# pathint/RankCompV3.jl

Hardware: AMD Instinct MI355X
Metric: gene-pair·sample comparisons/sec at 20k genes × 1k samples (higher is better)
Workload: dtype u16

## Files before the change

### rankcompv3.jl_amd/_ffi.py

```python
from __future__ import annotations

import ctypes
import os
import subprocess
from typing import NamedTuple

import numpy as np

_HERE = os.path.dirname(os.path.abspath(__file__))
LIB_PATH = os.environ.get("REO_LIB_PATH") or os.path.join(_HERE, "libreo_hip.so")
CSRC = os.path.join(_HERE, "csrc")

REO_OK, REO_EINVAL, REO_EHIP, REO_ECOMM, REO_ENOMEM = 0, -1, -2, -3, -4
NTIMINGS = 12

SYMBOLS = [
    "reo_version", "reo_last_error", "reo_create", "reo_destroy", "reo_trim_memory", "reo_set_shard", "reo_set_allreduce", "reo_set_allgather",
    "reo_create_multi", "reo_comm_unique_id", "reo_comm_init_rank",
    "reo_set_matrix_f64", "reo_set_matrix_i64", "reo_set_matrix_dev_f64", "reo_set_matrix_dev_i64",
    "reo_set_matrix_f32", "reo_set_matrix_i32", "reo_set_matrix_dev_f32", "reo_set_matrix_dev_i32",
    "reo_set_matrix_rm_f64", "reo_set_matrix_rm_i64", "reo_set_matrix_rm_f32", "reo_set_matrix_rm_i32",
    "reo_set_matrix_csc_f64", "reo_set_matrix_csc_i64", "reo_set_matrix_csc_f32", "reo_set_matrix_csc_i32",
    "reo_set_groups", "reo_compute_thresholds", "reo_set_thresholds", "reo_get_thresholds", "reo_threshold",
    "reo_build_pairs", "reo_pair_counts", "reo_get_codes", "reo_tally", "reo_identify_degs", "reo_mccullagh",
# ... 551 lines not shown
        out = np.zeros((cont.shape[0], 5), dtype=np.float64)
        check(self._L.reo_mccullagh(self._h, _ptr(cont), cont.shape[0], _ptr(out)))
        return out

    @staticmethod
    def _pseudobulk_args(cells, order, chunk_ptr):
        order = np.ascontiguousarray(order, dtype=np.int32)
        chunk_ptr = np.ascontiguousarray(chunk_ptr, dtype=np.int32)
        n_out = chunk_ptr.size - 1
        if hasattr(cells, "tocsc"):
            m = cells.tocsc()
            m.sort_indices()
            G, C = m.shape
            isint = np.issubdtype(m.dtype, np.integer)
            val = np.ascontiguousarray(m.data, dtype=np.int64 if isint else np.float64)
            colptr = np.ascontiguousarray(m.indptr, dtype=np.int64)
            rowidx = np.ascontiguousarray(m.indices, dtype=np.int32)
            args = (G, C, _ptr(colptr), _ptr(rowidx), _ptr(val), _ptr(order), order.size, _ptr(chunk_ptr), n_out)
            return "csc", "i64" if isint else "f64", args, G, (m, val, colptr, rowidx, order, chunk_ptr)
        X = np.asarray(cells)
        isint = np.issubdtype(X.dtype, np.integer)
        Xf = np.asfortranarray(X, dtype=np.int64 if isint else np.float64)
        G, C = Xf.shape
        args = (_ptr(Xf), G, C, G, _ptr(order), order.size, _ptr(chunk_ptr), n_out)
        return "dense", "i64" if isint else "f64", args, G, (Xf, order, chunk_ptr)

    def pseudobulk(self, cells, order, chunk_ptr) -> np.ndarray:
        form, ty, args, G, keep = self._pseudobulk_args(cells, order, chunk_ptr)
        out = np.zeros((G, args[-1]), dtype=np.int64 if ty == "i64" else np.float64, order="F")
        check(getattr(self._L, f"reo_pseudobulk_{form}_{ty}")(self._h, *args, _ptr(out)))
        return out

    def set_matrix_pseudobulk(self, cells, order, chunk_ptr) -> None:
        if is_device_sparse(cells) or is_device_tensor(cells):
            order = np.ascontiguousarray(order, dtype=np.int32)
            chunk_ptr = np.ascontiguousarray(chunk_ptr, dtype=np.int32)
            n_out = chunk_ptr.size - 1
            tail = (_ptr(order) if order.size else None, order.size, _ptr(chunk_ptr), n_out)
            if is_device_sparse(cells):
                ty, G, C, nnz, colptr, rowidx, val, bits, keep = device_csc_entry(cells)
                check(getattr(self._L, "reo_set_matrix_pseudobulk_csc_dev_" + ty)(self._h, G, C, nnz, _dptr(colptr), _dptr(rowidx), bits, _dptr(val), *tail))
            else:
                ptr, G, C, ld, ty, keep = device_matrix(cells)
                check(getattr(self._L, "reo_set_matrix_pseudobulk_dense_dev_" + ty)(self._h, ctypes.c_void_p(ptr), G, C, ld, *tail))
            self.G, self.S = G, n_out
            return
        form, ty, args, G, keep = self._pseudobulk_args(cells, order, chunk_ptr)
        check(getattr(self._L, f"reo_set_matrix_pseudobulk_{form}_{ty}")(self._h, *args))
        self.G, self.S = G, args[-1]

    def filter_matrix(self, min_profiles: int = 0, min_features: int = 0):
        info = self.info()
        pk = np.zeros(info["S"], dtype=np.uint8)
        gk = np.zeros(info["G"], dtype=np.uint8)
        sk, gkn = ctypes.c_int64(0), ctypes.c_int64(0)
        check(self._L.reo_filter_matrix(self._h, int(min_profiles), int(min_features), _ptr(pk) if pk.size else None, _ptr(gk) if gk.size else None,
                                        ctypes.byref(sk), ctypes.byref(gkn)))
        self.G, self.S = int(gkn.value), int(sk.value)
        return pk.astype(bool), gk.astype(bool)

    def get_matrix(self) -> np.ndarray:
        info = self.info()
        dt = {1: np.float64, 2: np.int64, 3: np.float32}.get(info["resident_dtype"])
        if dt is None:
            raise DimensionMismatch(REO_EINVAL, "no expression matrix set")
        out = np.zeros((info["G"], info["S"]), dtype=dt, order="F")
        check(self._L.reo_get_matrix(self._h, _ptr(out), out.nbytes))
        return out

    def set_profiling(self, on: bool) -> None:
        check(self._L.reo_set_profiling(self._h, 1 if on else 0))

    def reset_timings(self) -> None:
        check(self._L.reo_reset_timings(self._h))

    def timings(self) -> dict:
        ms = np.zeros(NTIMINGS, dtype=np.float64)
        check(self._L.reo_get_timings(self._h, _ptr(ms), NTIMINGS))
        return {"transform_ms": ms[0], "k1_ms": ms[1], "k2_ms": ms[2], "iter_ms": ms[3], "k3_ms": max(ms[3] - ms[2], 0.0), "k2_launches": int(ms[4]),
                "k1_launches": int(ms[5]), "exchange_ms": ms[6], "pseudobulk_ms": ms[7], "k2_full_ms": ms[8],
                "k2_full_launches": int(ms[9]), "k2_delta_ms": ms[10], "set_matrix_host_wall_ms": ms[11]}

    def info(self) -> dict:
        v = np.zeros(28, dtype=np.int64)
        check(self._L.reo_get_info(self._h, _ptr(v), 28))
        return {"G": int(v[0]), "S": int(v[1]), "Gp": int(v[2]), "table_bytes": int(v[3]), "has_ties": int(v[4]),
                "tiles_owned": int(v[5]), "tiles_total": int(v[6]), "tile_i": int(v[7]), "chunk_j": int(v[8]),
                "chunks_per_panel": int(v[9]), "unit_h": int(v[10]), "sample_slots": int(v[11]),
                "shared_group_counts": int(v[12]), "group_count_bytes": int(v[13]), "transform_in_lds": int(v[14]), "xcc_local_histograms": int(v[15]),
                "cycle_period": int(v[16]), "cycle_found_at_pass": int(v[17]), "cycle_passes_skipped": int(v[18]), "upload_link_bytes": int(v[19]),
                "eager_range_launches": int(v[20]), "rowmajor_upload": int(v[21]),
                "csc_upload": int(v[22]), "csc_nnz": int(v[23]), "resident_dtype": int(v[24]),
                "k1_slot_order": int(v[25]), "k1_half_tiles_separated": int(v[26]), "csc_device": int(v[27])}
```

### rankcompv3.jl_amd/csrc/api.hip

```cpp
#include <execinfo.h>
#include <signal.h>
#include <unistd.h>

#include <ctime>
#include <algorithm>
#include <chrono>
#include <cmath>
#include <cstdarg>
#include <cstdio>
#include <cstdlib>
#include <cstring>

#include "pair_list.h"
#include "reo_internal.h"
#include "sample_counts.h"
#include "upload_csc.h"

#include <mutex>
#include <unordered_map>

namespace reo {

static thread_local std::string g_err;
thread_local bool tl_release_synced = false;
// ... 503 lines not shown
    } else {
        set_error("the persistent iteration kernel gave up at a grid barrier (a workgroup did not arrive within its bound); "
                  "REO_LIGHT=1 runs the same passes as separate launches");
    }
    return REO_EHIP;
}

static int32_t need_complete_table(reo_ctx *c)
{
    if (c->built_k < 0) { set_error("no class table: call reo_build_pairs first"); return REO_EINVAL; }
    if (!c->table_complete) {
        set_error("shard %d of %d holds only its own part of the class table: attach a communicator (reo_comm_init_rank) or an "
                  "exchange hook (reo_set_allgather, reo_set_allreduce) before reo_build_pairs", c->rank, c->world);
        return REO_ECOMM;
    }
    return REO_OK;
}

}

using namespace reo;

extern "C" {

int32_t reo_version(void) { return 700; }

int32_t reo_trim_memory(void)
{
    std::vector<Block> all;
    {
        Pool &P = pool();
        std::lock_guard<std::mutex> lk(P.mu);
        all.swap(P.free_blocks);
        P.cached = 0;
    }
    int dev = 0;
    const bool have_dev = hipGetDevice(&dev) == hipSuccess;
    for (const Block &b : all) {
        if (!b.pinned) (void)hipSetDevice(b.device);
        raw_free(b.p, b.pinned);
    }
    {
        Handles &H = handles();
        std::lock_guard<std::mutex> lk(H.mu);
        for (int k = 0; k < 2; ++k) {
            for (auto &st : H.streams[k]) { (void)hipSetDevice(st.first); (void)hipStreamDestroy(st.second); }
            for (auto &ev : H.events[k]) { (void)hipSetDevice(ev.first); (void)hipEventDestroy(ev.second); }
            H.streams[k].clear(); H.events[k].clear();
        }
    }
    if (have_dev) (void)hipSetDevice(dev);
    return REO_OK;
}

const char *reo_last_error(void) { return g_err.c_str(); }

int32_t reo_create(reo_ctx **out, int32_t device, uint64_t seed)
{
    if (!out) { set_error("out is null"); return REO_EINVAL; }
    *out = nullptr;
    if (getenv("REO_DEBUG_SEGV")) install_segv_backtrace();
    int ndev = 0;
    if (hipGetDeviceCount(&ndev) != hipSuccess || ndev == 0) {
        set_error("no HIP device visible: libreo_hip has no CPU fallback");
        return REO_EHIP;
    }
    if (device < 0) REO_HIP_CHECK(hipGetDevice(&device));
    if (device >= ndev) { set_error("device %d out of range (%d visible)", device, ndev); return REO_EINVAL; }
    hipDeviceProp_t prop;
    REO_HIP_CHECK(hipGetDeviceProperties(&prop, device));
    if (strncmp(prop.gcnArchName, "gfx950", 6) != 0) {
        set_error("device %d is %s; this library carries gfx950 (MI355X) code objects only", device, prop.gcnArchName);
        return REO_EHIP;
    }
    REO_HIP_CHECK(hipSetDevice(device));
    reo_ctx *c = new (std::nothrow) reo_ctx();
    if (!c) { set_error("out of host memory"); return REO_ENOMEM; }
    c->device = device;
    c->seed = seed;
    if (const char *e = getenv("REO_K1_WAVE")) c->k1_wave = (e[0] != '0');
    if (const char *e = getenv("REO_K1_HALF")) c->k1_half = (e[0] != '0');
    if (const char *e = getenv("REO_K1_SLOTS")) c->k1_slots = (e[0] != '0');
    if (const char *e = getenv("REO_K1_QUEUE")) c->k1_queue = (e[0] != '0');
    if (const char *e = getenv("REO_K1_WORKERS")) c->k1_workers = std::max(1, atoi(e));
    if (const char *e = getenv("REO_K1_ORDER")) c->k1_order = std::max(0, std::min(2, atoi(e)));
    {
        int n = 0;
        if (hipDeviceGetAttribute(&n, hipDeviceAttributeMultiprocessorCount, c->device) == hipSuccess && n > 0) c->n_cus = n;
    }
    if (const char *e = getenv("REO_SPIN_WAIT")) c->spin_wait = (e[0] != '0');
    if (const char *e = getenv("REO_CHECK_HOOK_TABLE")) c->check_hook_table = (e[0] != '0');
    if (const char *e = getenv("REO_SHARE_GROUP_COUNTS")) c->share_counts = (e[0] != '0');
    if (const char *e = getenv("REO_LIGHT_BAND")) c->light_band = std::max(0, atoi(e));
    if (const char *e = getenv("REO_HIST_BELOW")) c->hist_below = std::max(0, atoi(e));
    if (const char *e = getenv("REO_CYCLE")) c->cycle_watch = atoi(e) != 0;
    if (const char *e = getenv("REO_LIGHT")) c->light_mode = e[0] == '0' ? 0 : (e[0] == '2' ? 2 : (e[0] == '3' ? 3 : 1));
    c->light_window = light_window(); c->light_min_g = light_min_genes();
    if (const char *e = getenv("REO_LIGHT_WINDOW")) c->light_window = std::max(1, std::min(31, atoi(e)));
    if (const char *e = getenv("REO_LIGHT_MIN_G")) c->light_min_g = std::max(64, atoi(e));
    if (const char *e = getenv("REO_STATE_MIRROR")) c->state_mirror_wanted = (e[0] != '0');
    if (const char *e = getenv("REO_EXCHANGE_WAVES")) c->x_waves = std::max(1, std::min(8, atoi(e)));
    if (const char *e = getenv("REO_EAGER_UPLOAD")) c->eager_mode = std::max(0, std::min(2, atoi(e)));
    if (const char *e = getenv("REO_EAGER_CHUNK")) c->eager_chunk = std::max(1, atoi(e));
    if (const char *e = getenv("REO_EAGER_GATE")) c->eager_gate = atoi(e) != 0;
    if (const char *e = getenv("REO_EAGER_RANGES")) c->eager_ranges = std::max(1, std::min(6, atoi(e)));
    if (const char *e = getenv("REO_UPLOAD_THREADS")) c->upload_threads = std::max(0, std::min(64, atoi(e)));
    c->debug_passes = getenv("REO_DEBUG_PASSES") != nullptr;
    c->debug_stamps = getenv("REO_DEBUG_STAMPS") != nullptr;
    c->k1_stamps = getenv("REO_K1_STAMPS") != nullptr;
    hipError_t e = handle_stream(&c->stream, 0);
    if (e != hipSuccess) { delete c; set_error("hipStreamCreate failed: %s", hipGetErrorString(e)); return REO_EHIP; }
    int ok = 0;
    const char *xe = getenv("REO_XCC_LOCAL");
    if (!(xe && xe[0] == '0')) {
        const int32_t rc = xcc_selftest(c, &ok);
        if (rc) { reo_destroy(c); return rc; }
    }
    c->xcc_local = ok;
    *out = c;
    return REO_OK;
}

void reo_destroy(reo_ctx *c)
{
    if (!c) return;
    for (reo_ctx *p : c->peers) reo_destroy(p);
    c->peers.clear();
    (void)hipSetDevice(c->device);
    for (int q = 0; q < 2; ++q) if (c->k1s[q]) (void)hipStreamSynchronize(c->k1s[q]);
    if (c->xs) (void)hipStreamSynchronize(c->xs);
    if (c->up) (void)hipStreamSynchronize(c->up);
    if (c->rk) (void)hipStreamSynchronize(c->rk);
    (void)hipStreamSynchronize(c->stream);
    comm_release(c);
    collect_timings(c);
    tl_release_synced = true;
    for (auto &t : c->pool) { release_event(t.a, 1); release_event(t.b, 1); }
    c->dX_owned.release(); c->pos.release(); c->lo.release(); c->hi.release(); c->goff_dev.release();
    c->table.release();
    c->t_kin.release(); c->t_kout.release(); c->t_vin.release(); c->t_vout.release(); c->t_temp.release();
    c->t_order.release(); c->t_flags.release(); c->t_slots.release(); c->unit_map.release();
    for (auto &il : c->k1_wave_items) il.buf.release();
    for (int q = 0; q < 2; ++q) { release_stream(c->k1s[q], 0); release_event(c->ev_k1_join[q], 0); }
    release_stream(c->xs, 0);
    release_stream(c->up, 0);
    release_stream(c->rk, 1);
    for (auto &e : c->ev_rk) release_event(e, 0);
    for (auto &e : c->ev_up) release_event(e, 0);
    c->e_lists.release();
    for (int q = 0; q < 3; ++q) {
        if (c->stage_h[q]) pool_free(c->stage_h[q], c->stage_cap, true);
        c->stage_d[q].release();
        release_event(c->ev_stage[q], 0);
        release_event(c->ev_widen[q], 0);
    }
    release_event(c->ev_fork, 0);
    release_event(c->ev_x, 0);
    for (auto &e : c->ev_k1) release_event(e, 0);
    c->t_pos16.release(); c->t_lo16.release(); c->t_hi16.release(); c->gcounts.release();
    c->k1_slot_part.release(); c->k1_slot_maps.release(); c->pos_s.release(); c->lo_s.release(); c->k1_queue_ctr.release();
    c->t_pos32.release(); c->t_lo32.release(); c->t_hi32.release(); c->t_vin32.release(); c->t_vout32.release();
    for (int t = 0; t < 2; ++t) { c->refbits[t].release(); c->refbytes[t].release(); }
    c->raw.release(); c->delta_list.release(); c->cont.release(); c->result.release(); c->sorted_d.release(); c->sorted_p.release();
    c->rank_s.release(); c->rank_a.release(); c->scal.release(); c->blockmin.release();
    c->state.release(); c->trace.release(); c->modes.release(); c->cand.release(); c->hist.release(); c->mrank.release(); c->lstate.release(); c->clist.release(); c->olist.release(); c->units_all.release(); c->xsend.release(); c->xrecv.release(); c->check_flag.release(); c->gridbar.release(); c->chunk_v.release(); c->chunk_i.release(); c->part.release();
    if (c->host_state) pool_free(c->host_state, sizeof(IterState), true);
// ... 707 lines not shown
    } else {
        maskbits = c->refbits[c->ref_slot].p;
    }
    DrainOnExit drain(c);
    if (map != c->sc_slot2col_host || c->sc_slot2col.p != c->sc_slot2col_uploaded) {
        c->sc_slot2col_host = map;
        c->sc_slot2col_uploaded = nullptr;
        REO_HIP_CHECK(hipMemcpyAsync(c->sc_slot2col.p, c->sc_slot2col_host.data(), map.size() * sizeof(int32_t), hipMemcpyHostToDevice, c->stream));
        c->sc_slot2col_uploaded = c->sc_slot2col.p;
    }
    if (partner_mask) {
        REO_HIP_CHECK(hipMemsetAsync(d_maskbytes.p, 0, c->Gp, c->stream));
        REO_HIP_CHECK(hipMemcpyAsync(d_maskbytes.p, partner_mask, static_cast<size_t>(c->G), hipMemcpyHostToDevice, c->stream));
        if ((rc = launch_pack_ref(c, d_maskbytes.p, d_maskbits.p))) return rc;
    }
    for (int64_t q0 = 0; q0 < n_genes; q0 += batch) {
        const int64_t nq = std::min(batch, n_genes - q0);
        const size_t rows = static_cast<size_t>(nq) * static_cast<size_t>(S);
        REO_HIP_CHECK(hipMemcpyAsync(d_genes.p, genes + q0, static_cast<size_t>(nq) * sizeof(int32_t), hipMemcpyHostToDevice, c->stream));
        if ((rc = launch_sample_counts(c, d_genes.p, nq, maskbits, class_mask, c->sc_slot2col.p, d_sel.p, d_gt.p, n_eq ? d_eq.p : nullptr))) return rc;
        REO_HIP_CHECK(hipMemcpyAsync(n_gt + static_cast<size_t>(q0) * S, d_gt.p, rows * sizeof(int32_t), hipMemcpyDeviceToHost, c->stream));
        if (n_eq) REO_HIP_CHECK(hipMemcpyAsync(n_eq + static_cast<size_t>(q0) * S, d_eq.p, rows * sizeof(int32_t), hipMemcpyDeviceToHost, c->stream));
        if (n_sel) REO_HIP_CHECK(hipMemcpyAsync(n_sel + q0, d_sel.p, static_cast<size_t>(nq) * sizeof(int32_t), hipMemcpyDeviceToHost, c->stream));
        if ((rc = wait_or_drop_table(c))) return rc;
    }
    drain.dismiss();
    return REO_OK;
}

int32_t reo_mccullagh(reo_ctx *c, const int32_t *cont, int64_t n, double *out)
{
    int32_t rc = use(c);
    if (rc) return rc;
    if (!cont || !out || n < 1) { set_error("bad argument"); return REO_EINVAL; }
    DevBuf<int32_t> dc;
    DevBuf<double> dout;
    if ((rc = dc.ensure(n * 9)) || (rc = dout.ensure(n * 5))) return rc;
    DrainOnExit drain(c);
    hipError_t e = hipMemcpyAsync(dc.p, cont, sizeof(int32_t) * 9 * n, hipMemcpyHostToDevice, c->stream);
    if (e == hipSuccess) {
        rc = launch_mccullagh(c, dc.p, n, dout.p);
        if (!rc) {
            e = hipMemcpyAsync(out, dout.p, sizeof(double) * 5 * n, hipMemcpyDeviceToHost, c->stream);
            if (e == hipSuccess) e = hipStreamSynchronize(c->stream);
        }
    }
    if (e != hipSuccess) { set_error("HIP failure: %s", hipGetErrorString(e)); rc = REO_EHIP; }
    dc.release(); dout.release();
    return rc;
}

int32_t reo_set_profiling(reo_ctx *c, int32_t on)
{
    if (!c) { set_error("null context"); return REO_EINVAL; }
    c->profiling = on != 0;
    for (reo_ctx *p : c->peers) p->profiling = c->profiling;
    return REO_OK;
}

int32_t reo_reset_timings(reo_ctx *c)
{
    if (!c) { set_error("null context"); return REO_EINVAL; }
    collect_timings(c);
    for (double &v : c->t_ms) v = 0.0;
    return REO_OK;
}

int32_t reo_get_timings(reo_ctx *c, double *ms, int32_t n)
{
    if (!c || !ms) { set_error("null argument"); return REO_EINVAL; }
    collect_timings(c);
    for (int i = 0; i < n && i < REO_NTIMINGS; ++i) ms[i] = c->t_ms[i];
    return REO_OK;
}

int32_t reo_get_info(reo_ctx *c, int64_t *info, int32_t n)
{
    if (!c || !info) { set_error("null argument"); return REO_EINVAL; }
    int64_t separated = 0;
    if (n > 26 && c->last_k1_slots) {
        int32_t rc = use(c);
        if (rc || (rc = launch_slot_separated(c, &separated))) return rc;
    }
    const int64_t v[28] = {c->G, c->S, c->Gp, static_cast<int64_t>(c->table.n * sizeof(uint32_t)), c->has_ties,
                           c->tiles_owned, c->tiles_total, kTileI, c->k1_cj, c->k1_q, kUnitH,
                           c->goff32.empty() ? 0 : c->goff32.back(), c->last_k1_shared,
                           static_cast<int64_t>(c->gcounts.n * sizeof(uint16_t)), c->transform_in_lds, c->xcc_local,
                           c->it_cycle_period, c->it_cycle_at, c->it_cycle_skipped, c->narrowed_bytes, c->eager_range_launches, c->rowmajor_upload,
                           c->csc_upload, c->csc_nnz, c->dtype, c->last_k1_slots, separated, c->csc_device};
    for (int i = 0; i < n && i < 28; ++i) info[i] = v[i];
    return REO_OK;
}

}
```

### rankcompv3.jl_amd/csrc/k1_slots.h

```cpp
#pragma once

#include <cstddef>
#include <cstdint>

#if defined(__HIPCC__) || defined(__CUDACC__)
#define REO_SLOTS_HD __host__ __device__ inline
#else
#define REO_SLOTS_HD inline
#endif

namespace reo {

constexpr int kSlotTile = 32;
constexpr int kSlotChunk = 256;
constexpr uint32_t kSlotNoMin = 0xFFFFu, kSlotNoMax = 0u;

REO_SLOTS_HD uint32_t slot_pack(uint32_t mn, uint32_t mx) { return mn | mx << 16; }
REO_SLOTS_HD uint32_t slot_min(uint32_t w) { return w & 0xFFFFu; }
REO_SLOTS_HD uint32_t slot_max(uint32_t w) { return w >> 16; }
REO_SLOTS_HD uint32_t slot_join(uint32_t a, uint32_t b)
{
    const uint32_t mn = slot_min(a) < slot_min(b) ? slot_min(a) : slot_min(b), mx = slot_max(a) > slot_max(b) ? slot_max(a) : slot_max(b);
    return slot_pack(mn, mx);
}

REO_SLOTS_HD uint32_t slot_key(uint32_t side0, uint32_t side1) { return slot_min(side0) + slot_max(side0) + slot_min(side1) + slot_max(side1); }

REO_SLOTS_HD uint64_t slot_order_key(uint32_t key, uint32_t gene) { return static_cast<uint64_t>(key) << 32 | gene; }

REO_SLOTS_HD int slot_separated(uint32_t tile_rng, uint32_t chunk_rng)
{
    if (slot_max(chunk_rng) < slot_min(tile_rng)) return 1;
    if (slot_max(tile_rng) < slot_min(chunk_rng)) return -1;
    return 0;
}

REO_SLOTS_HD int slot_item_tile(uint32_t item) { return static_cast<int>(item & 0x3FFFu); }
REO_SLOTS_HD int slot_item_chunk(uint32_t item) { return static_cast<int>((item >> 16) & 0x7FFFu); }
REO_SLOTS_HD int slot_item_side(uint32_t item) { return static_cast<int>(item >> 31); }
REO_SLOTS_HD int slot_item_halves(uint32_t item) { return (item & 0x8000u) ? 1 : 2; }


inline void slot_rank(const uint32_t *key, int G, uint32_t *g2s)
{
    for (int g = 0; g < G; ++g) {
        uint32_t n = 0;
        for (int h = 0; h < G; ++h) n += slot_order_key(key[h], static_cast<uint32_t>(h)) < slot_order_key(key[g], static_cast<uint32_t>(g)) ? 1u : 0u;
        g2s[g] = n;
    }
}

inline void slot_invert(const uint32_t *g2s_G, int G, int Gp, uint32_t *g2s, uint32_t *s2g)
{
    for (int g = 0; g < G; ++g) { g2s[g] = g2s_G[g]; s2g[g2s_G[g]] = static_cast<uint32_t>(g); }
    for (int g = G; g < Gp; ++g) g2s[g] = s2g[g] = static_cast<uint32_t>(g);
}

inline void slot_unpermute_row(const uint32_t *in, uint32_t *out, int W, const uint32_t *g2s, int G)
{
    for (int w = 0; w < W; ++w) out[w] = 0;
    for (int j = 0; j < G; ++j) {
        const uint32_t k = g2s[j];
        out[j >> 5] |= ((in[k >> 5] >> (k & 31)) & 1u) << (j & 31);
    }
}

inline void slot_permute_row(const uint32_t *in, uint32_t *out, int W, const uint32_t *s2g, int G)
{
    for (int w = 0; w < W; ++w) out[w] = 0;
    for (int k = 0; k < G; ++k) {
        const uint32_t j = s2g[k];
        out[k >> 5] |= ((in[j >> 5] >> (j & 31)) & 1u) << (k & 31);
    }
}

}
```

### rankcompv3.jl_amd/csrc/kernels.hip

```cpp
#include <algorithm>
#include <chrono>
#include <cstddef>
#include <cstdio>
#include <cstdlib>
#include <cstring>
#include <mutex>
#include <type_traits>

#include "reo_internal.h"
#include "k1_items.h"
#include "k1_slots.h"
#include "k1_queue.h"

namespace reo {

namespace {

__device__ __forceinline__ uint64_t mix64(uint64_t z)
{
    z += 0x9E3779B97F4A7C15ULL;
    z = (z ^ (z >> 30)) * 0xBF58476D1CE4E5B9ULL;
    z = (z ^ (z >> 27)) * 0x94D049BB133111EBULL;
    return z ^ (z >> 31);
}
// ... 607 lines not shown

__global__ __launch_bounds__(256) void k1_slot_invert(uint32_t *__restrict__ g2s, uint32_t *__restrict__ s2g, int G, int Gp)
{
    const int g = blockIdx.x * 256 + threadIdx.x;
    if (g >= Gp) return;
    if (g < G) { const uint32_t k = g2s[g]; if (k < static_cast<uint32_t>(G)) s2g[k] = static_cast<uint32_t>(g); }
    else { g2s[g] = static_cast<uint32_t>(g); s2g[g] = static_cast<uint32_t>(g); }
}

__global__ __launch_bounds__(256) void k1_slot_ranges(const uint32_t *__restrict__ gmm, const uint32_t *__restrict__ s2g, int G, int Gp,
                                                      uint32_t *__restrict__ trng, uint32_t *__restrict__ crng)
{
    static_assert(kSlotTile == kTileI && kSlotChunk == 64 * kRJ, "k1_slots.h carries its own copy of the item geometry");
    __shared__ uint32_t sm[8];
    const int k = blockIdx.x * 256 + threadIdx.x, side = blockIdx.y;
    uint32_t r = k < G ? gmm[static_cast<size_t>(side) * Gp + s2g[k]] : slot_pack(kSlotNoMin, kSlotNoMax);
#pragma unroll
    for (int o = 1; o < 32; o <<= 1) r = slot_join(r, static_cast<uint32_t>(__shfl_xor(static_cast<int>(r), o)));
    if ((threadIdx.x & 31) == 0) { trng[static_cast<size_t>(side) * (Gp >> 5) + (k >> 5)] = r; sm[threadIdx.x >> 5] = r; }
    __syncthreads();
    if (threadIdx.x == 0) {
        for (int q = 1; q < 8; ++q) r = slot_join(r, sm[q]);
        crng[static_cast<size_t>(side) * (Gp >> 8) + blockIdx.x] = r;
    }
}

__global__ __launch_bounds__(256) void k1_slot_gather(const uint4 *__restrict__ P, const uint4 *__restrict__ AL, const uint32_t *__restrict__ s2g, int Gp,
                                                      uint4 *__restrict__ Ps, uint4 *__restrict__ ALs)
{
    const int k = blockIdx.x * 256 + threadIdx.x, b = blockIdx.y;
    const uint32_t g = s2g[k];
#pragma unroll
    for (int q = 0; q < 4; ++q) Ps[(static_cast<size_t>(b) * 4 + q) * Gp + k] = P[(static_cast<size_t>(b) * 4 + q) * Gp + g];
#pragma unroll
    for (int e = 0; e < 4; ++e) {
        const int kk = blockIdx.x * 256 + e * 64 + (threadIdx.x >> 2), q = threadIdx.x & 3;
        ALs[(static_cast<size_t>(b) * Gp + kk) * 4 + q] = AL[(static_cast<size_t>(b) * Gp + s2g[kk]) * 4 + q];
    }
}

template <int R>
__global__ __launch_bounds__(256) void k1_unslot_columns(uint32_t *__restrict__ table, const uint32_t *__restrict__ g2s, int G, int Wp)
{
    extern __shared__ uint4 unslot_sm[];
    uint32_t *sm = reinterpret_cast<uint32_t *>(unslot_sm);
    const int r0 = blockIdx.x * R, nr = min(R, G - r0);
    if (nr <= 0) return;
    uint32_t *rows = table + static_cast<size_t>(r0) * kPlanes * Wp;
    for (int rp = 0; rp < nr * kPlanes; ++rp)
        for (int w = threadIdx.x; w < Wp; w += 256) sm[(static_cast<size_t>(rp >> 2) * Wp + w) * 4 + (rp & 3)] = rows[static_cast<size_t>(rp) * Wp + w];
    __syncthreads();
    for (int wo = threadIdx.x; wo < Wp; wo += 256) {
        uint32_t acc[R][4];
#pragma unroll
        for (int r = 0; r < R; ++r) acc[r][0] = acc[r][1] = acc[r][2] = acc[r][3] = 0;
        const uint4 *kq = reinterpret_cast<const uint4 *>(g2s) + static_cast<size_t>(wo) * 8;
#pragma unroll 2
        for (int i = 0; i < 8; ++i) {
            const uint4 k4 = kq[i];
            const uint32_t ks[4] = {k4.x, k4.y, k4.z, k4.w};
#pragma unroll
            for (int e = 0; e < 4; ++e) {
                const uint32_t k = ks[e], kw = min(k >> 5, static_cast<uint32_t>(Wp - 1)), kb = k & 31u;
#pragma unroll
                for (int r = 0; r < R; ++r) {
                    if (r < nr) {
                        const uint4 w = unslot_sm[static_cast<size_t>(r) * Wp + kw];
                        acc[r][0] = __builtin_amdgcn_alignbit(w.x >> kb, acc[r][0], 1);
                        acc[r][1] = __builtin_amdgcn_alignbit(w.y >> kb, acc[r][1], 1);
                        acc[r][2] = __builtin_amdgcn_alignbit(w.z >> kb, acc[r][2], 1);
                        acc[r][3] = __builtin_amdgcn_alignbit(w.w >> kb, acc[r][3], 1);
                    }
                }
            }
        }
        const int left = G - 32 * wo;
        const uint32_t valid = left >= 32 ? 0xFFFFFFFFu : (left <= 0 ? 0u : (1u << left) - 1u);
#pragma unroll
        for (int r = 0; r < R; ++r)
            if (r < nr) {
#pragma unroll
                for (int pl = 0; pl < 4; ++pl) rows[(static_cast<size_t>(r) * kPlanes + pl) * Wp + wo] = acc[r][pl] & valid;
            }
    }
}

__global__ __launch_bounds__(256) void k1_slot_count(const uint32_t *__restrict__ items, int n, const uint32_t *__restrict__ trng, const uint32_t *__restrict__ crng,
                                                     int Gp, unsigned long long *__restrict__ out)
{
    const int i = blockIdx.x * 256 + threadIdx.x;
    int v = 0;
    if (i < n) {
        const uint32_t it = items[i];
        const int side = slot_item_side(it);
        if (slot_separated(trng[static_cast<size_t>(side) * (Gp >> 5) + slot_item_tile(it)], crng[static_cast<size_t>(side) * (Gp >> 8) + slot_item_chunk(it)]))
            v = slot_item_halves(it);
    }
    const unsigned long long m1 = __ballot(v == 1), m2 = __ballot(v == 2);
    if ((threadIdx.x & 63) == 0 && (m1 | m2)) atomicAdd(out, static_cast<unsigned long long>(__builtin_popcountll(m1) + 2 * __builtin_popcountll(m2)));
}

template <int NB>
__global__ __launch_bounds__(64, NB > 16 ? 2 : 3) void k1w_pairs_gated(K1Args a)
{
    constexpr int RI = kTileI;
    constexpr int ROWB = NB > 16 ? 128 : 64;
    __shared__ uint4 ring[2 * RI * ROWB / 16];
    const int bad = a.gate[0] | a.gate[4] | a.gate[5], ties = a.gate[1];
    if (bad) return;
    if (ties) k1w_body<NB, true>(a, ring, blockIdx.x);
    else k1w_body<NB, false>(a, ring, blockIdx.x);
}

constexpr int kRJWide = 2, kRJWideTies = 1;

template <int RJ, int NB, bool TIES>
__device__ __forceinline__ void count_pass_wide(const uint4 *__restrict__ P, const uint4 *__restrict__ AL, const uint4 *__restrict__ AH,
                                                int Gp, int i0, int jl, int bb, int be, uint32_t (&gt)[RJ][kTileI],
                                                uint32_t (&ge)[TIES ? RJ : 1][kTileI], uint4 *sm_lo, uint4 *sm_hi, bool idle)
{
    static_assert((TIES && RJ == 1) || (!TIES && RJ == 2), "four chains per bit plane");
    constexpr int RI = kTileI, NQ = (NB + 3) / 4;
    constexpr int kStageQ = kStageB * RI * 4;
    constexpr int kPerThread = kStageQ / 256;
#pragma unroll
    for (int r = 0; r < RJ; ++r)
#pragma unroll
        for (int ii = 0; ii < RI; ++ii) { gt[r][ii] = 0; if (TIES) ge[r][ii] = 0; }
    if (bb >= be) return;
    uint4 sl[kPerThread], sh[TIES ? kPerThread : 1];
    auto stage_load = [&](int b0) {
#pragma unroll
        for (int e = 0; e < kPerThread; ++e) {
            const int idx = threadIdx.x + 256 * e;
            const int b = min(b0 + idx / (RI * 4), be - 1);
            const size_t o = (static_cast<size_t>(b) * Gp + i0) * 4 + idx % (RI * 4);
            sl[e] = AL[o];
            if (TIES) sh[e] = AH[o];
        }
    };
    auto stage_store = [&](int buf) {
#pragma unroll
        for (int e = 0; e < kPerThread; ++e) {
            sm_lo[buf * kStageQ + threadIdx.x + 256 * e] = sl[e];
            if (TIES) sm_hi[buf * kStageQ + threadIdx.x + 256 * e] = sh[e];
        }
    };
    stage_load(bb);
    __syncthreads();
    stage_store(0);
    __syncthreads();
    int buf = 0;
    for (int b0 = bb; b0 < be; b0 += kStageB) {
        const bool more = b0 + kStageB < be;
        if (more) stage_load(b0 + kStageB);
        const int nb = idle ? 0 : min(kStageB, be - b0);
        for (int s = 0; s < nb; ++s) {
            Planes16 p[RJ];
#pragma unroll
            for (int r = 0; r < RJ; ++r)
#pragma unroll
                for (int q = 0; q < NQ; ++q) p[r].set(q, P[(static_cast<size_t>(b0 + s) * 4 + q) * Gp + jl + 64 * r]);
            const uint4 *al = sm_lo + buf * kStageQ + s * RI * 4;
            const uint4 *ah = sm_hi + buf * kStageQ + s * RI * 4;
#pragma clang loop unroll(full)
            for (int i = 0; i < RI; i += 2) {
// ... 2878 lines not shown
    int32_t rc;
    if ((rc = c->unit_map.ensure(std::max<size_t>(units.size(), 1)))) return rc;
    if (!units.empty() && (c->unit_map.p != c->unit_map_uploaded || units != c->unit_map_host)) {
        REO_HIP_CHECK(hipMemcpyAsync(c->unit_map.p, units.data(), units.size() * sizeof(uint32_t), hipMemcpyHostToDevice, c->stream));
        REO_HIP_CHECK(hipStreamSynchronize(c->stream));
        c->unit_map_host = units;
        c->unit_map_uploaded = c->unit_map.p;
    }
    return REO_OK;
}

static int32_t apply_range(reo_ctx *c, K1Args &a, int sides, const K1Range *range, size_t n_items)
{
    int32_t rc;
    const int side = sides == 1 ? 0 : 1, sb = side ? a.tb : a.cb, se = side ? a.te : a.ce;
    if (range->b0 < 0 || range->b1 <= range->b0 || sb + range->b1 > se || (range->first != (range->b0 == 0)) || (range->last != (sb + range->b1 == se))) {
        set_error("a range of sample blocks outside its side"); return REO_EINVAL;
    }
    if (!(range->first && range->last)) {
        if ((rc = c->k1_park[side].ensure(std::max<size_t>(n_items, 1) * kParkSlot)) || (rc = c->k1_park_ge[side].ensure(std::max<size_t>(n_items, 1)))) return rc;
        a.park = c->k1_park[side].p; a.park_ge = c->k1_park_ge[side].p;
        a.park_mode = (range->first ? 0 : 1) | (range->last ? 0 : 2);
    }
    (side ? a.tb : a.cb) = sb + range->b0;
    (side ? a.te : a.ce) = sb + range->b1;
    return REO_OK;
}


struct SlotMaps { uint32_t *gmm, *key, *g2s, *s2g, *trng, *crng; unsigned long long *count; };
static size_t slot_maps_words(int Gp) { return static_cast<size_t>(Gp) * 5 + static_cast<size_t>(Gp) / 16 + static_cast<size_t>(Gp) / 128 + 2; }
static SlotMaps slot_maps(const reo_ctx *c)
{
    SlotMaps m;
    const size_t Gp = static_cast<size_t>(c->Gp);
    m.gmm = c->k1_slot_maps.p; m.key = m.gmm + 2 * Gp; m.g2s = m.key + Gp; m.s2g = m.g2s + Gp;
    m.trng = m.s2g + Gp; m.crng = m.trng + Gp / 16;
    m.count = reinterpret_cast<unsigned long long *>(m.crng + Gp / 128);
    return m;
}

static bool k1_slots_wanted(const reo_ctx *c, const K1Plan &pl, int sides, bool keep_table, const int32_t *gate, const K1Range *range, bool prepare)
{
    return c->k1_slots && pl.wave && !pl.wide && !pl.big && c->ngroups == 2 && sides == 3 && !c->has_ties && c->world == 1 && !c->in_multi &&
           !gate && !range && !prepare && !keep_table && c->t_pos16.p && c->t_pos16.n >= static_cast<size_t>(c->goff32[2]) * c->Gp;
}

static int32_t k1_slots_alloc(reo_ctx *c)
{
    int32_t rc;
    const size_t nq = static_cast<size_t>(c->goff32[2] / 32) * c->Gp * 4;
    if ((rc = c->k1_slot_part.ensure(static_cast<size_t>(kSlotSplits) * 2 * c->Gp)) || (rc = c->k1_slot_maps.ensure(slot_maps_words(c->Gp))) ||
        (rc = c->pos_s.ensure(nq)) || (rc = c->lo_s.ensure(nq)))
        return rc;
    if (c->k1_queue && c->k1_queue_ctr.ensure(kQueueWords)) (void)hipGetLastError();
    return REO_OK;
}

static int32_t k1_slots_front(reo_ctx *c, K1Args &a)
{
    const int G = a.G, Gp = a.Gp, nblk = c->goff32[2] / 32;
    const SlotMaps m = slot_maps(c);
    const unsigned gb = static_cast<unsigned>((G + 255) / 256);
    REO_HIP_CHECK(hipMemsetAsync(m.g2s, 0, static_cast<size_t>(Gp) * 2 * sizeof(uint32_t), c->stream));
    k1_slot_part<<<dim3(gb, kSlotSplits, 2), 256, 0, c->stream>>>(c->t_pos16.p, Gp, G, a.cb * 32, a.nc, a.tb * 32, a.nt, c->k1_slot_part.p);
    k1_slot_keys<<<gb, 256, 0, c->stream>>>(c->k1_slot_part.p, Gp, G, m.gmm, m.key);
    k1_slot_rank<<<dim3(gb, static_cast<unsigned>((G + kSlotRankSpan - 1) / kSlotRankSpan)), 256, 0, c->stream>>>(m.key, G, m.g2s);
    k1_slot_invert<<<static_cast<unsigned>(Gp / 256), 256, 0, c->stream>>>(m.g2s, m.s2g, G, Gp);
    k1_slot_ranges<<<dim3(static_cast<unsigned>(Gp / 256), 2), 256, 0, c->stream>>>(m.gmm, m.s2g, G, Gp, m.trng, m.crng);
    k1_slot_gather<<<dim3(static_cast<unsigned>(Gp / 256), static_cast<unsigned>(nblk)), 256, 0, c->stream>>>(c->pos.p, c->lo.p, m.s2g, Gp, c->pos_s.p, c->lo_s.p);
    REO_HIP_CHECK(hipGetLastError());
    a.P = c->pos_s.p; a.AL = c->lo_s.p; a.AH = c->lo_s.p;
    a.s2g = m.s2g; a.trng = m.trng; a.crng = m.crng;
    a.n_items = static_cast<uint32_t>(c->k1_items_n);
    if (c->k1_queue && c->k1_queue_ctr.p && c->k1_queue_ctr.n >= static_cast<size_t>(kQueueWords)) {
        REO_HIP_CHECK(hipMemsetAsync(c->k1_queue_ctr.p, 0, kQueueWords * sizeof(uint32_t), c->stream));
        a.queue = c->k1_queue_ctr.p;
    }
    return REO_OK;
}

static int32_t k1_slots_back(reo_ctx *c, const K1Args &a)
{
    const size_t row_bytes = static_cast<size_t>(a.Wp) * 16;
    auto go = [&](auto rtag) {
        constexpr int R = decltype(rtag)::value;
        k1_unslot_columns<R><<<static_cast<unsigned>((a.G + R - 1) / R), 256, R * row_bytes, c->stream>>>(a.table, slot_maps(c).g2s, a.G, a.Wp);
    };
    if (6 * row_bytes <= 61440) go(std::integral_constant<int, 6>{});
    else if (4 * row_bytes <= 61440) go(std::integral_constant<int, 4>{});
    else if (2 * row_bytes <= 61440) go(std::integral_constant<int, 2>{});
    else go(std::integral_constant<int, 1>{});
    REO_HIP_CHECK(hipGetLastError());
    return REO_OK;
}

int32_t launch_slot_separated(reo_ctx *c, int64_t *half_tiles)
{
    *half_tiles = 0;
    if (!c->last_k1_slots || !c->k1_slot_items || !c->k1_slot_items_n || !c->k1_slot_maps.p) return REO_OK;
    const reo_ctx::ItemList &il = c->k1_wave_items[0];
    if (c->k1_slot_gp != c->Gp || c->k1_slot_maps.n < slot_maps_words(c->Gp) || c->k1_slot_items != il.buf.p || c->k1_slot_items_n > il.buf.n) return REO_OK;
    const SlotMaps m = slot_maps(c);
    unsigned long long n = 0;
    REO_HIP_CHECK(hipMemsetAsync(m.count, 0, sizeof n, c->stream));
    k1_slot_count<<<static_cast<unsigned>((c->k1_slot_items_n + 255) / 256), 256, 0, c->stream>>>(c->k1_slot_items, static_cast<int>(c->k1_slot_items_n), m.trng, m.crng, c->Gp, m.count);
    REO_HIP_CHECK(hipGetLastError());
    REO_HIP_CHECK(hipMemcpyAsync(&n, m.count, sizeof n, hipMemcpyDeviceToHost, c->stream));
    REO_HIP_CHECK(hipStreamSynchronize(c->stream));
    *half_tiles = static_cast<int64_t>(n);
    return REO_OK;
}

int32_t launch_k1(reo_ctx *c, int k, int sides, bool keep_table, const int32_t *gate, const K1Range *range, bool prepare)
{
    K1Args a = k1_args(c, k);
    K1Plan pl;
    int32_t rc;
    if ((rc = k1_plan(c, sides, pl))) return rc;
    const std::vector<uint32_t> &units = pl.units;
    c->units_all_host = pl.units_all;
    c->tiles_owned = pl.tiles_owned; c->tiles_total = pl.tiles_total;
    c->k1_cj = pl.CJ; c->k1_q = pl.Q;
    a.n_units = static_cast<int>(units.size()); a.Q = pl.Q;
    if ((rc = upload_unit_map(c, units))) return rc;
    a.unit_map = c->unit_map.p;
    a.gate = gate;
    if (!prepare) { c->last_k1_slots = 0; c->k1_slot_items = nullptr; c->k1_slot_items_n = 0; c->k1_slot_gp = 0; }
    if ((range || prepare) && (sides != 1 && sides != 2)) { set_error("a range of sample blocks / a prepared launch: one side of the pair kernel"); return REO_EINVAL; }
    if (gate && (!pl.wave || pl.wide || pl.big)) { set_error("a gated launch of the pair kernel: wave form, at most 65535 genes and samples"); return REO_EINVAL; }
    c->x_pipelined = false;
    const int maxu_x = exchange_units_per_rank(c);
    const int nwaves = (pl.wave && sides == 3 && c->world > 1 && (c->comm || c->ag) && !c->in_multi && !c->k1_stamps) ? std::min({c->x_waves, 8, maxu_x}) : 1;
    if (nwaves > 1) {
        hipStream_t main_stream = c->stream;
        return pipelined_exchange(c, a, pl, nwaves, maxu_x, [&](int w, hipStream_t ks) {
            c->stream = ks;
            a.items = c->k1_wave_items[w].buf.p; c->k1_items_n = c->k1_wave_items[w].n;
            if (c->k1_items_n) dispatch_pairs(c, a, pl);
            c->stream = main_stream;
        });
    }
    if (pl.wave || (pl.wcounts && !c->gc_valid) || pl.wmulti) {
        reo_ctx::ItemList &il = c->k1_wave_items[sides == 3 ? 0 : sides];
        const auto w0 = std::chrono::steady_clock::now();
        if ((rc = item_list(c, a, pl, sides, units, il, 0, 1))) return rc;
        if (c->debug_passes) fprintf(stderr, "  launch_k1 sides %d: item list (%zu items) ready after %.0f us\n", sides, il.n, std::chrono::duration<double, std::micro>(std::chrono::steady_clock::now() - w0).count());
        a.items = il.buf.p; c->k1_items_n = il.n;
        if (prepare) return REO_OK;
        if (range && (rc = apply_range(c, a, sides, range, il.n))) return rc;
        if (c->k1_stamps) REO_HIP_CHECK(hipMalloc(reinterpret_cast<void **>(&a.stamps), (std::max<size_t>(c->k1_items_n, 1) * 4 + 2) * sizeof(unsigned long long)));
    }
    if (!keep_table) {
        if (!c->table_prezeroed) REO_HIP_CHECK(hipMemsetAsync(c->table.p, 0, static_cast<size_t>(c->G) * kPlanes * c->Wp * sizeof(uint32_t), c->stream));
        c->table_prezeroed = false;
    }
    if (units.empty()) return REO_OK;
    c->last_k1_shared = pl.shared ? 1 : 0;
    if (k1_slots_wanted(c, pl, sides, keep_table, gate, range, prepare) && c->k1_items_n) {
        if (k1_slots_alloc(c) == REO_OK) pl.slots = true;
        else (void)hipGetLastError();
    }
    if (a.stamps) k_time_mark<<<1, 64, 0, c->stream>>>(a.stamps + c->k1_items_n * 4);
    tic(c, 1);
    if (pl.slots && (rc = k1_slots_front(c, a))) { toc(c); return rc; }
    dispatch_pairs(c, a, pl);
// ... 298 lines not shown
```

### rankcompv3.jl_amd/csrc/reo_internal.h

```cpp
#pragma once

#include <hip/hip_runtime.h>

#include <cstdint>
#include <functional>
#include <string>
#include <vector>

#include "reo_hip.h"

namespace reo {

constexpr int kTileJ = 256;
constexpr int kTileI = 32;
constexpr int kPlanes = 4;
constexpr int kUnitH = 32;
constexpr int kRJ = 4;
constexpr int kRJTies = 2;
constexpr int kMaxGenes = 262143;
constexpr int kGenePad = 1024;
constexpr int kRaw = 8;
constexpr int kDeltaMax = 128;
constexpr int kSortChunk = 1024;

// ... 121 lines not shown

struct reo_ctx {
    int device = 0;
    hipStream_t stream = nullptr;
    uint64_t seed = 0;
    int rank = 0, world = 1;
    reo_allreduce_fn ar = nullptr;
    void *ar_user = nullptr;
    reo_allgather_fn ag = nullptr;
    void *ag_user = nullptr;

    int64_t G = 0, S = 0, ld = 0;
    int dtype = 0;
    const void *dX = nullptr;
    reo::DevBuf<unsigned char> dX_owned;
    std::vector<int32_t> group_id;
    int ngroups = 0;
    std::vector<int32_t> thr;
    bool thr_set = false;

    int Gp = 0, Wp = 0;
    std::vector<int32_t> goff;
    std::vector<int32_t> goff32;
    reo::DevBuf<uint4> pos;
    reo::DevBuf<uint4> lo;
    reo::DevBuf<uint4> hi;
    reo::DevBuf<uint16_t> t_pos16, t_lo16, t_hi16;
    reo::DevBuf<uint32_t> t_pos32, t_lo32, t_hi32;
    reo::DevBuf<uint32_t> t_vin32, t_vout32;
    reo::DevBuf<int32_t> goff_dev;
    reo::DevBuf<uint64_t> t_kin, t_kout;
    reo::DevBuf<uint16_t> t_vin, t_vout;
    reo::DevBuf<unsigned char> t_temp;
    reo::DevBuf<int32_t> t_order, t_flags, t_slots;
    reo::DevBuf<uint32_t> unit_map;
    std::vector<uint32_t> unit_map_host;
    std::vector<int32_t> t_order_host, t_slots_host, goff_blocks_host;
    const int32_t *t_meta_ptr[3] = {nullptr, nullptr, nullptr};
    int32_t *host_flags = nullptr;
    hipEvent_t ev_flags = nullptr;
    bool table_prezeroed = false;
    const uint32_t *unit_map_uploaded = nullptr;
    size_t k1_items_n = 0;
    bool transformed = false;
    int eager_mode = 2;
    int eager_chunk = 0;
    int eager_gate = 1;
    hipStream_t up = nullptr, rk = nullptr;
    hipEvent_t ev_up[8] = {nullptr};
    hipEvent_t ev_rk[4] = {nullptr, nullptr, nullptr, nullptr};
    reo::DevBuf<int32_t> e_lists;
    int upload_threads = 12;
    unsigned char *stage_h[3] = {nullptr, nullptr, nullptr};
    size_t stage_cap = 0;
    reo::DevBuf<unsigned char> stage_d[3];
    hipEvent_t ev_stage[3] = {nullptr, nullptr, nullptr}, ev_widen[3] = {nullptr, nullptr, nullptr};
    int64_t narrowed_bytes = 0;
    int rowmajor_upload = 0;
    int csc_upload = 0;
    int64_t csc_nnz = 0;
    reo::DevBuf<int64_t> csc_colptr;
    int csc_device = 0;
    bool eager_k1 = false;
    int has_ties = 0;
    int transform_in_lds = 0;

    reo::DevBuf<uint32_t> table;
    int built_k = -1;
    bool table_complete = false;
    void *comm = nullptr;
    int spin_wait = 0;
    int check_hook_table = 1;
    bool comm_dead = false;
    bool in_multi = false;
    bool multi_one_device = false;
    std::vector<reo_ctx *> peers;
    reo::DevBuf<uint16_t> gcounts;
    bool gc_valid = false;
    int k1_wave = 1;
    int k1_order = 0;
    int k1_half = 1;
    int k1_slots = 1;
    int last_k1_slots = 0;
    const uint32_t *k1_slot_items = nullptr;
    size_t k1_slot_items_n = 0;
    int k1_slot_gp = 0;
    reo::DevBuf<uint32_t> k1_slot_part;
    reo::DevBuf<uint32_t> k1_slot_maps;
    reo::DevBuf<uint4> pos_s, lo_s;
    int k1_queue = 1;
    int k1_workers = 0;
    reo::DevBuf<uint32_t> k1_queue_ctr;
    int n_cus = 256;
    int share_counts = 1;
    int last_k1_shared = 0;
    int64_t tiles_owned = 0, tiles_total = 0;
    int k1_cj = 0, k1_q = 0;
    std::vector<uint32_t> units_all_host, units_all_dev;
    const uint32_t *units_all_uploaded = nullptr;
    reo::DevBuf<uint32_t> units_all, xsend, xrecv;
    int x_waves = 4;
    bool x_pipelined = false;
    hipStream_t k1s[2] = {nullptr, nullptr}, xs = nullptr;
    hipEvent_t ev_fork = nullptr, ev_k1[8] = {nullptr}, ev_k1_join[2] = {nullptr, nullptr}, ev_x = nullptr;
    struct ItemList { reo::DevBuf<uint32_t> buf; size_t n = 0; uint64_t key[5] = {0, 0, 0, 0, 0}; };
    ItemList k1_wave_items[8];
    reo::DevBuf<uint32_t> k1_park[2];
    reo::DevBuf<int32_t> k1_park_ge[2];
    int64_t eager_range_launches = 0;
    int eager_ranges = -1;
    reo::DevBuf<int32_t> check_flag;

    reo::DevBuf<uint32_t> refbits[2];
    reo::DevBuf<uint8_t> refbytes[2];
    int ref_slot = -1;
    const char *ref_gone = "reo_identify_degs has not run on this context";
    reo::DevBuf<int32_t> sc_slot2col;
    std::vector<int32_t> sc_slot2col_host;
    const int32_t *sc_slot2col_uploaded = nullptr;
    reo::DevBuf<int32_t> raw;
    reo::DevBuf<uint32_t> delta_list;
    reo::DevBuf<int32_t> cont;
    reo::DevBuf<double> result;
    reo::DevBuf<double> sorted_d;
    reo::DevBuf<double> sorted_p;
    reo::DevBuf<uint32_t> rank_s, rank_a;
    reo::DevBuf<double> scal;
    reo::DevBuf<double> blockmin;
    reo::DevBuf<double> chunk_v;
    reo::DevBuf<uint16_t> chunk_i;
    reo::DevBuf<double> part;
    reo::DevBuf<reo::IterState> state;
    reo::DevBuf<int32_t> trace;
    reo::DevBuf<int32_t> modes;
    reo::DevBuf<double> cand;
    reo::DevBuf<unsigned> gridbar;
    reo::DevBuf<reo::LightState> lstate;
    reo::DevBuf<int32_t> clist;
    int light_band = 32;
    bool cycle_watch = true;
    reo::DevBuf<uint8_t> snap;
    int it_cycle_period = 0, it_cycle_at = 0, it_cycle_skipped = 0;
    int hist_below = 256;
    int xcc_local = 0;
    int light_window = 24, light_min_g = 4096;
    int light_mode = 1;
    reo::DevBuf<int32_t> olist;
    reo::DevBuf<int32_t> hist, mrank;
    double it_pval_deg = 1.0, it_padj_deg = 0.05;
    int it_n_iter = 0, it_n_conv = 0, it_a0 = 0, it_b0 = 0;
    int k2_idx = 0;
    int it_light_form = 1;
    bool it_no_light = false;
    reo::IterState *host_state = nullptr;
    bool state_mirror_wanted = true;
    bool debug_passes = false, debug_stamps = false, k1_stamps = false;
    bool state_mirror = false;
    uint8_t *host_ref = nullptr;
    size_t host_ref_cap = 0;

    bool profiling = false;
    double t_ms[REO_NTIMINGS] = {0};
    std::vector<std::pair<int, reo::StageTimer>> pending;
    std::vector<reo::StageTimer> pool;
    std::vector<size_t> open;
    std::vector<int32_t> k2_modes;
// ... 72 lines not shown
```

Baseline: 44920 billion.

## Unslot K1 table columns via LDS bit-transpose with gathered word rebuild

Replaces the per-row column unpermute after slot-ordered K1 with a kernel that bit-transposes whole packed words of R rows into a padded LDS bitmap. Each output word is then rebuilt by gathering 32 slot bits through g2s and transposing back. The goal is to cut the per-bit scalar permutation cost and raise parallelism with up to 1024 threads per block. It uses up to 160 KB of dynamic LDS and an attribute call on first use, which limits occupancy. A wide or narrow form is picked from Gp and can be overridden by an environment variable.

```diff
diff --git a/rankcompv3.jl_amd/_ffi.py b/rankcompv3.jl_amd/_ffi.py
--- a/rankcompv3.jl_amd/_ffi.py
+++ b/rankcompv3.jl_amd/_ffi.py
@@ -657,8 +657,10 @@
                 "k2_full_launches": int(ms[9]), "k2_delta_ms": ms[10], "set_matrix_host_wall_ms": ms[11]}
 
     def info(self) -> dict:
+        w = np.zeros(29, dtype=np.int64)
+        check(self._L.reo_get_info(self._h, _ptr(w), 29))
         v = np.zeros(28, dtype=np.int64)
-        check(self._L.reo_get_info(self._h, _ptr(v), 28))
+        v[:] = w[:28]
         return {"G": int(v[0]), "S": int(v[1]), "Gp": int(v[2]), "table_bytes": int(v[3]), "has_ties": int(v[4]),
                 "tiles_owned": int(v[5]), "tiles_total": int(v[6]), "tile_i": int(v[7]), "chunk_j": int(v[8]),
                 "chunks_per_panel": int(v[9]), "unit_h": int(v[10]), "sample_slots": int(v[11]),
@@ -666,4 +668,5 @@
                 "cycle_period": int(v[16]), "cycle_found_at_pass": int(v[17]), "cycle_passes_skipped": int(v[18]), "upload_link_bytes": int(v[19]),
                 "eager_range_launches": int(v[20]), "rowmajor_upload": int(v[21]),
                 "csc_upload": int(v[22]), "csc_nnz": int(v[23]), "resident_dtype": int(v[24]),
-                "k1_slot_order": int(v[25]), "k1_half_tiles_separated": int(v[26]), "csc_device": int(v[27])}
+                "k1_slot_order": int(v[25]), "k1_half_tiles_separated": int(v[26]), "csc_device": int(v[27]),
+                "k1_unslot_form": int(w[28])}
diff --git a/rankcompv3.jl_amd/csrc/api.hip b/rankcompv3.jl_amd/csrc/api.hip
--- a/rankcompv3.jl_amd/csrc/api.hip
+++ b/rankcompv3.jl_amd/csrc/api.hip
@@ -609,6 +609,7 @@
     if (const char *e = getenv("REO_K1_HALF")) c->k1_half = (e[0] != '0');
     if (const char *e = getenv("REO_K1_SLOTS")) c->k1_slots = (e[0] != '0');
     if (const char *e = getenv("REO_K1_QUEUE")) c->k1_queue = (e[0] != '0');
+    if (const char *e = getenv("REO_K1_UNSLOT")) { const int v = atoi(e); c->k1_unslot = (v == 8 || v == 4) ? v : (e[0] == '0' ? 0 : -1); }
     if (const char *e = getenv("REO_K1_WORKERS")) c->k1_workers = std::max(1, atoi(e));
     if (const char *e = getenv("REO_K1_ORDER")) c->k1_order = std::max(0, std::min(2, atoi(e)));
     {
@@ -1482,14 +1483,15 @@
         int32_t rc = use(c);
         if (rc || (rc = launch_slot_separated(c, &separated))) return rc;
     }
-    const int64_t v[28] = {c->G, c->S, c->Gp, static_cast<int64_t>(c->table.n * sizeof(uint32_t)), c->has_ties,
+    const int64_t v[29] = {c->G, c->S, c->Gp, static_cast<int64_t>(c->table.n * sizeof(uint32_t)), c->has_ties,
                            c->tiles_owned, c->tiles_total, kTileI, c->k1_cj, c->k1_q, kUnitH,
                            c->goff32.empty() ? 0 : c->goff32.back(), c->last_k1_shared,
                            static_cast<int64_t>(c->gcounts.n * sizeof(uint16_t)), c->transform_in_lds, c->xcc_local,
                            c->it_cycle_period, c->it_cycle_at, c->it_cycle_skipped, c->narrowed_bytes, c->eager_range_launches, c->rowmajor_upload,
-                           c->csc_upload, c->csc_nnz, c->dtype, c->last_k1_slots, separated, c->csc_device};
-    for (int i = 0; i < n && i < 28; ++i) info[i] = v[i];
-    return REO_OK;
-}
-
-}
+                           c->csc_upload, c->csc_nnz, c->dtype, c->last_k1_slots, separated, c->csc_device,
+                           c->last_k1_slots ? c->last_k1_unslot : 0};
+    for (int i = 0; i < n && i < 29; ++i) info[i] = v[i];
+    return REO_OK;
+}
+
+}
diff --git a/rankcompv3.jl_amd/csrc/k1_slots.h b/rankcompv3.jl_amd/csrc/k1_slots.h
--- a/rankcompv3.jl_amd/csrc/k1_slots.h
+++ b/rankcompv3.jl_amd/csrc/k1_slots.h
@@ -65,6 +65,112 @@
     }
 }
 
+constexpr int kUnslotWide = 8, kUnslotNarrow = 4;
+constexpr size_t kUnslotLdsLimit = 160 * 1024;
+constexpr int kUnslotThreadsMax = 1024;
+
+REO_SLOTS_HD int unslot_bit(int row, int plane) { return 4 * row + plane; }
+
+REO_SLOTS_HD uint32_t unslot_lds_index(int form, uint32_t k)
+{
+    const uint32_t w = k >> 5, b = k & 31u;
+    return form == kUnslotWide ? 33u * w + b : 2u * (17u * w + (b & 15u)) + (b >> 4);
+}
+
+REO_SLOTS_HD size_t unslot_lds_bytes(int form, int Gp) { return static_cast<size_t>(Gp / 32) * (form == kUnslotWide ? 33u * 4u : 17u * 4u); }
+
+REO_SLOTS_HD int unslot_form(int Gp)
+{
+    if (3 * unslot_lds_bytes(kUnslotNarrow, Gp) <= kUnslotLdsLimit) return kUnslotNarrow;
+    return unslot_lds_bytes(kUnslotWide, Gp) <= kUnslotLdsLimit ? kUnslotWide : kUnslotNarrow;
+}
+
+REO_SLOTS_HD int unslot_threads(int Wp)
+{
+    const int trips = (Wp + kUnslotThreadsMax - 1) / kUnslotThreadsMax;
+    return ((Wp + trips - 1) / trips + 63) / 64 * 64;
+}
+
+#if defined(__clang__)
+#define REO_SLOTS_UNROLL _Pragma("unroll")
+#else
+#define REO_SLOTS_UNROLL
+#endif
+
+template <int N>
+REO_SLOTS_HD void unslot_transpose(uint32_t (&w)[N])
+{
+    static_assert(N == 32 || N == 16, "4 R words");
+    uint32_t m = N == 32 ? 0x0000FFFFu : 0x00FF00FFu;
+    REO_SLOTS_UNROLL
+    for (int j = N / 2; j != 0; j >>= 1, m ^= (m << j)) {
+        REO_SLOTS_UNROLL
+        for (int k = 0; k < N; k = (k + j + 1) & ~j) {
+            const uint32_t t = ((w[k] >> j) ^ w[k + j]) & m;
+            w[k] ^= t << j;
+            w[k + j] ^= t;
+        }
+    }
+}
+
+template <int R>
+REO_SLOTS_HD void unslot_in_word(uint32_t (&m)[4 * R], int w, uint32_t *T)
+{
+    unslot_transpose<4 * R>(m);
+    if (R == kUnslotWide) {
+        REO_SLOTS_UNROLL
+        for (int b = 0; b < 4 * R; ++b) T[unslot_lds_index(R, 32u * w + b)] = m[b];
+    } else {
+        REO_SLOTS_UNROLL
+        for (int i = 0; i < 4 * R; ++i) T[unslot_lds_index(R, 32u * w + i) >> 1] = m[i];
+    }
+}
+
+template <int R>
+REO_SLOTS_HD void unslot_out_word(uint32_t (&u)[4 * R], const uint32_t (&ks)[32], int wo, const uint32_t *T, int G, int Gp)
+{
+    if (R == kUnslotWide) {
+        REO_SLOTS_UNROLL
+        for (int c = 0; c < 32; ++c) {
+            const uint32_t k = ks[c] < static_cast<uint32_t>(Gp) ? ks[c] : static_cast<uint32_t>(Gp - 1);
+            u[c % (4 * R)] = T[unslot_lds_index(R, k)];
+        }
+    } else {
+        const uint16_t *T16 = reinterpret_cast<const uint16_t *>(T);
+        REO_SLOTS_UNROLL
+        for (int c = 0; c < 32; ++c) {
+            const uint32_t k = ks[c] < static_cast<uint32_t>(Gp) ? ks[c] : static_cast<uint32_t>(Gp - 1);
+            const uint32_t e = T16[unslot_lds_index(R, k)];
+            if (c < 16) u[c % (4 * R)] = e;
+            else u[c % (4 * R)] |= e << 16;
+        }
+    }
+    unslot_transpose<4 * R>(u);
+    const int left = G - 32 * wo;
+    const uint32_t valid = left >= 32 ? 0xFFFFFFFFu : (left <= 0 ? 0u : (1u << left) - 1u);
+    REO_SLOTS_UNROLL
+    for (int q = 0; q < 4 * R; ++q) u[q] &= valid;
+}
+
+template <int R>
+inline void unslot_group_model(uint32_t *table, int r0, int n_rows, int G, int Wp, const uint32_t *g2s, uint32_t *T)
+{
+    const int nr = n_rows - r0 < R ? n_rows - r0 : R;
+    if (nr <= 0) return;
+    uint32_t *rows = table + static_cast<size_t>(r0) * 4 * Wp;
+    for (int w = 0; w < Wp; ++w) {
+        uint32_t m[4 * R];
+        for (int q = 0; q < 4 * R; ++q) m[q] = q < 4 * nr ? rows[static_cast<size_t>(q) * Wp + w] : 0u;
+        unslot_in_word<R>(m, w, T);
+    }
+    for (int wo = 0; wo < Wp; ++wo) {
+        uint32_t u[4 * R], ks[32];
+        for (int c = 0; c < 32; ++c) ks[c] = g2s[32 * wo + c];
+        unslot_out_word<R>(u, ks, wo, T, G, 32 * Wp);
+        for (int q = 0; q < 4 * nr; ++q) rows[static_cast<size_t>(q) * Wp + wo] = u[q];
+    }
+}
+
 inline void slot_permute_row(const uint32_t *in, uint32_t *out, int W, const uint32_t *s2g, int G)
 {
     for (int w = 0; w < W; ++w) out[w] = 0;
diff --git a/rankcompv3.jl_amd/csrc/kernels.hip b/rankcompv3.jl_amd/csrc/kernels.hip
--- a/rankcompv3.jl_amd/csrc/kernels.hip
+++ b/rankcompv3.jl_amd/csrc/kernels.hip
@@ -713,6 +713,37 @@
 #pragma unroll
                 for (int pl = 0; pl < 4; ++pl) rows[(static_cast<size_t>(r) * kPlanes + pl) * Wp + wo] = acc[r][pl] & valid;
             }
+    }
+}
+
+template <int R>
+__global__ __launch_bounds__(kUnslotThreadsMax) void k1_unslot_words(uint32_t *__restrict__ table, const uint32_t *__restrict__ g2s, int G, int Wp)
+{
+    constexpr int NQ = 4 * R;
+    extern __shared__ uint32_t unslot_t[];
+    const int r0 = blockIdx.x * R, nr = min(R, G - r0);
+    if (nr <= 0) return;
+    const int nq = nr * kPlanes;
+    uint32_t *rows = table + static_cast<size_t>(r0) * kPlanes * Wp;
+    for (int w = threadIdx.x; w < Wp; w += blockDim.x) {
+        uint32_t m[NQ];
+#pragma unroll
+        for (int q = 0; q < NQ; ++q) m[q] = q < nq ? rows[static_cast<size_t>(q) * Wp + w] : 0u;
+        unslot_in_word<R>(m, w, unslot_t);
+    }
+    __syncthreads();
+    for (int wo = threadIdx.x; wo < Wp; wo += blockDim.x) {
+        const uint4 *kq = reinterpret_cast<const uint4 *>(g2s) + static_cast<size_t>(wo) * 8;
+        uint32_t ks[32], u[NQ];
+#pragma unroll
+        for (int i = 0; i < 8; ++i) {
+            const uint4 k4 = kq[i];
+            ks[4 * i] = k4.x; ks[4 * i + 1] = k4.y; ks[4 * i + 2] = k4.z; ks[4 * i + 3] = k4.w;
+        }
+        unslot_out_word<R>(u, ks, wo, unslot_t, G, 32 * Wp);
+#pragma unroll
+        for (int q = 0; q < NQ; ++q)
+            if (q < nq) rows[static_cast<size_t>(q) * Wp + wo] = u[q];
     }
 }
 
@@ -3757,6 +3788,29 @@
 
 static int32_t k1_slots_back(reo_ctx *c, const K1Args &a)
 {
+    if (c->k1_unslot != 0) {
+        int form = unslot_form(a.Gp);
+        if ((c->k1_unslot == kUnslotWide || c->k1_unslot == kUnslotNarrow) && unslot_lds_bytes(c->k1_unslot, a.Gp) <= kUnslotLdsLimit) form = c->k1_unslot;
+        const size_t lds = unslot_lds_bytes(form, a.Gp);
+        if (lds <= kUnslotLdsLimit) {
+            auto go = [&](auto rtag) -> int32_t {
+                constexpr int R = decltype(rtag)::value;
+                const int bit = R == kUnslotWide ? 1 : 2;
+                if (!(c->k1_unslot_attr & bit)) {
+                    REO_HIP_CHECK(hipFuncSetAttribute(reinterpret_cast<const void *>(k1_unslot_words<R>), hipFuncAttributeMaxDynamicSharedMemorySize, static_cast<int>(kUnslotLdsLimit)));
+                    c->k1_unslot_attr |= bit;
+                }
+                k1_unslot_words<R><<<static_cast<unsigned>((a.G + R - 1) / R), static_cast<unsigned>(unslot_threads(a.Wp)), lds, c->stream>>>(a.table, slot_maps(c).g2s, a.G, a.Wp);
+                return REO_OK;
+            };
+            const int32_t rc = form == kUnslotWide ? go(std::integral_constant<int, kUnslotWide>{}) : go(std::integral_constant<int, kUnslotNarrow>{});
+            if (rc) return rc;
+            REO_HIP_CHECK(hipGetLastError());
+            c->last_k1_unslot = form;
+            return REO_OK;
+        }
+    }
+    c->last_k1_unslot = 1;
     const size_t row_bytes = static_cast<size_t>(a.Wp) * 16;
     auto go = [&](auto rtag) {
         constexpr int R = decltype(rtag)::value;
diff --git a/rankcompv3.jl_amd/csrc/reo_internal.h b/rankcompv3.jl_amd/csrc/reo_internal.h
--- a/rankcompv3.jl_amd/csrc/reo_internal.h
+++ b/rankcompv3.jl_amd/csrc/reo_internal.h
@@ -227,6 +227,9 @@
     int k1_half = 1;
     int k1_slots = 1;
     int last_k1_slots = 0;
+    int k1_unslot = -1;
+    int last_k1_unslot = 0;
+    int k1_unslot_attr = 0;
     const uint32_t *k1_slot_items = nullptr;
     size_t k1_slot_items_n = 0;
     int k1_slot_gp = 0;
```

Result: faster. 49140 billion (median of 6 runs) (+9.4%).
